# jkflying/opencalibration

Measured on AMD Instinct MI355X. Metric: images/sec end-to-end (extract+match+relax) on synthetic aerial grid; LM iters/sec, higher is better.
Workload: dtype f32 (extract) + fp4 0/1 bits, f32 accumulate, exact (match) + f64 (RANSAC, relax)

## Files before the change

opencalibration_amd/capi.py:

```python
import ctypes as C
import os

import numpy as np

_HERE = os.path.dirname(os.path.abspath(__file__))
LIB_PATH = os.path.join(_HERE, "libochip.so")

K_MATCH, K_RANSAC, K_RELAX_EVAL, K_RELAX_SOLVE, K_AKAZE = 0, 1, 2, 3, 4
NO_SECOND = 0xFFFF

PAIR_DTYPE = np.dtype([("image_1", np.uint32), ("image_2", np.uint32)])
MATCH_DTYPE = np.dtype([("best_k", np.uint32), ("best_count", np.uint16), ("second_count", np.uint16)])
RANSAC_JOB_DTYPE = np.dtype([("image_1", np.uint32), ("image_2", np.uint32), ("n", np.uint32), ("rng_state", np.uint32),
                             ("match_offset", np.uint64), ("eval_offset", np.uint64)])
RANSAC_MATCH_DTYPE = np.dtype([("k1", np.uint32), ("k2", np.uint32), ("count", np.uint16), ("reserved", np.uint16)])
RANSAC_RESULT_DTYPE = np.dtype([("H", np.float64, (9,)), ("score", np.float64), ("iterations", np.uint32), ("n_inliers", np.uint32),
                                ("improvements", np.uint32), ("reserved", np.uint32)])

EXPORTS = [
    "ochip_ctx_create", "ochip_ctx_destroy", "ochip_ctx_sibling", "ochip_ctx_attachment", "ochip_akaze_progress", "ochip_ctx_set_priority", "ochip_last_error", "ochip_device_info", "ochip_synchronize",
    "ochip_descriptors_reserve", "ochip_upload_descriptors", "ochip_descriptor_count",
    "ochip_match_batch", "ochip_match_launch", "ochip_match_fetch",
    "ochip_upload_keypoints", "ochip_ransac_homography_batch", "ochip_refit_homography_batch", "ochip_ransac_epipolar_batch",
    "ochip_upload_batch", "ochip_host_alloc", "ochip_host_free", "ochip_akaze_batch", "ochip_akaze_batch_dev", "ochip_akaze_features", "ochip_akaze_features_dev", "ochip_feature_lists_from_keypoints",
# ... 285 lines not shown

    def std_sort(self, keys, payload, offsets):
        keys = np.ascontiguousarray(keys, np.uint32)
        payload = np.ascontiguousarray(payload, np.uint32)
        offsets = np.ascontiguousarray(offsets, np.uint32)
        n_segs = len(offsets) - 1
        ko, po = np.zeros(max(len(keys), 1), np.uint32), np.zeros(max(len(keys), 1), np.uint32)
        fb = np.zeros(max(n_segs, 1), np.uint8)
        kin = keys if len(keys) else np.zeros(1, np.uint32)
        pin = payload if len(keys) else np.zeros(1, np.uint32)
        self._check(self.L.ochip_debug_std_sort(self.h, kin.ctypes.data, pin.ctypes.data, offsets.ctypes.data, n_segs, ko.ctypes.data,
                                                po.ctypes.data, fb.ctypes.data), "ochip_debug_std_sort")
        return ko[:len(keys)], po[:len(keys)], fb[:n_segs].astype(bool)

    def feature_lists(self, kp6, desc, work_wh, scale, nms_radius=8.0, subset_spacing=0.0):
        kp6 = np.ascontiguousarray(kp6, np.float32).reshape(-1, 6)
        desc = np.ascontiguousarray(desc, np.uint64).reshape(-1, 8)
        n = len(kp6)
        m = max(n, 1)
        rec, resp = np.zeros((m + 1, 88), np.uint8), np.zeros(m, np.float32)
        slot, ns, conflict = np.zeros(m, np.uint32), np.zeros(4, np.uint32), np.zeros(16, np.uint8)
        subset, nsub, sconf = np.zeros(16384, np.uint32), np.zeros(4, np.uint32), np.zeros(16, np.uint8)
        counts = np.array([n], np.uint32)

        class Lists(C.Structure):
            _fields_ = [("records", C.c_void_p), ("response", C.c_void_p), ("slot", C.c_void_p), ("num_sparse", C.c_void_p),
                        ("conflict", C.c_void_p), ("subset", C.c_void_p), ("num_subset", C.c_void_p), ("subset_conflict", C.c_void_p),
                        ("subset_spacing", C.c_double)]

        lists = Lists(rec.ctypes.data, resp.ctypes.data, slot.ctypes.data, ns.ctypes.data, conflict.ctypes.data, subset.ctypes.data,
                      nsub.ctypes.data, sconf.ctypes.data, float(subset_spacing))
        kin = kp6 if n else np.zeros((1, 6), np.float32)
        din = desc if n else np.zeros((1, 8), np.uint64)
        self._check(self.L.ochip_feature_lists_from_keypoints(self.h, kin.ctypes.data, din.ctypes.data, counts.ctypes.data, 1, m,
                                                              int(work_wh[0]), int(work_wh[1]), float(scale), float(nms_radius),
                                                              C.byref(lists)), "ochip_feature_lists_from_keypoints")
        out = dict(records=rec[:n + 1 if n else 0], response=resp[:n], slot=slot[:n], num_sparse=int(ns[0]), conflict=bool(conflict[0]))
        if subset_spacing > 0:
            out.update(subset=subset[:int(nsub[0])].copy(), subset_conflict=bool(sconf[0]))
        return out

    def synth_views(self, position, orientation, width, height, f, pp, plane, spacing, origin, seed=7, chunk=64):
        n = len(position)
        ptr = C.c_void_p()
        self._check(self.L.ochip_synth_views_alloc(self.h, n, width, height, C.byref(ptr)), "ochip_synth_views_alloc")
        cams = np.ascontiguousarray(np.concatenate([position, orientation], axis=1), np.float64)
        model3 = np.array([f, pp[0], pp[1]], np.float64)
        plane2 = np.array(plane, np.float64)
        lat3 = np.array([origin[0], origin[1], spacing], np.float64)
        for i in range(0, n, chunk):
            m = min(chunk, n - i)
            c = np.ascontiguousarray(cams[i:i + m])
            self._check(self.L.ochip_synth_render_views(self.h, ptr, i, m, width, height, c.ctypes.data, model3.ctypes.data,
                                                        plane2.ctypes.data, lat3.ctypes.data, seed), "ochip_synth_render_views")
        return ptr.value
# ... 195 lines not shown
```

opencalibration_amd/csrc/akaze.hip:

```cpp
#include "ctx.hpp"

#include <algorithm>
#include <cmath>
#include <limits>
#include <cstring>
#include <type_traits>
#include <vector>

namespace
{

struct level_info
{
    int octave, w, h, sigma_size;
    float esigma;
    size_t off;
    int tile_off, tiles_x;
    int mask_off;
    int sup_off, sup_tx;
};

__device__ __forceinline__ int clampi(int v, int lo, int hi)
{
    return v < lo ? lo : (v > hi ? hi : v);
}
__device__ __forceinline__ int reflect101_once(int v, int n)
{
    v = v < 0 ? -v : v;
    return v >= n ? 2 * (n - 1) - v : v;
}
__device__ __forceinline__ int reflect101(int v, int n)
// ... 740 lines not shown
__global__ void copy_plane_kernel(const float *__restrict__ in, size_t in_stride, float *__restrict__ out,
                                  size_t out_stride, size_t n)
{
    const size_t i = (size_t)blockIdx.x * blockDim.x + threadIdx.x;
    if (i < n)
        out[(size_t)blockIdx.z * out_stride + i] = in[(size_t)blockIdx.z * in_stride + i];
}

struct cand_t
{
    int level, x, y;
    float response;
    float dx, dy;
};

template <int S>
__global__ __launch_bounds__(256) void det_maxima_kernel(const float2 *__restrict__ Lxy, size_t stride,
                                                         float2 *__restrict__ Fit, float *__restrict__ Rmax, int w, int h,
                                                         float thr, unsigned int *__restrict__ tile_counts, int tile_off,
                                                         int n_tiles, float margin, unsigned long long *__restrict__ mask,
                                                         size_t mask_stride)
{
    constexpr int HW = S + 1, RW = BT_X + 2 * HW, RH = DT_Y + 2 * HW, DW = BT_X + 2, DH = DT_Y + 2;
    __shared__ float tx[RW * RH], ty[RW * RH];
    static_assert(DW * DH <= RW * RH, "the determinant tile reuses the Lx tile's storage");
    float *td = tx;
    const int tiles_x = (w + BT_X - 1) / BT_X, tiles_y = (h + DT_Y - 1) / DT_Y;
    int tile_x, tile_y;
    if (!xcd_tile(tiles_x, tiles_y, &tile_x, &tile_y))
        return;
    const int x0 = tile_x * BT_X, y0 = tile_y * DT_Y;
    const int rx0 = x0 - HW, ry0 = y0 - HW;
    const float2 *XY = Lxy + (size_t)blockIdx.z * stride;
// ... 154 lines not shown
                            mx = false;
                if (mx)
                {
                    out = v;
                    const float vxp = td[ci + 1], vxm = td[ci - 1], vyp = td[ci + DW], vym = td[ci - DW];
                    const float Dx = 0.5f * (vxp - vxm), Dy = 0.5f * (vyp - vym);
                    const float Dxx = (vxp + vxm) - 2.0f * v, Dyy = (vyp + vym) - 2.0f * v;
                    const float Dxy = 0.25f * ((td[ci + DW + 1] + td[ci - DW - 1]) - (td[ci + DW - 1] + td[ci - DW + 1]));
                    fit = subpixel_solve(Dxx, Dxy, Dyy, Dx, Dy);
                }
            }
        }
        const unsigned long long m = __ballot(out != 0.0f);
        if (out != 0.0f)
        {
            Rmax[(size_t)blockIdx.z * stride + (size_t)y * w + x] = out;
            Fit[(size_t)blockIdx.z * stride + (size_t)y * w + x] = fit;
        }
        if (lx == 0 && y < h)
        {
            mask[(size_t)blockIdx.z * mask_stride + (size_t)y * tiles_x + tile_x] = m;
            found += (unsigned int)__popcll(m);
        }
    }
    __shared__ unsigned int wsum[4];
    for (int off = 32; off >= 1; off >>= 1)
        found += (unsigned int)__shfl_xor((int)found, off);
    if ((threadIdx.x & 63) == 0)
        wsum[threadIdx.x >> 6] = found;
    __syncthreads();
    if (threadIdx.x == 0)
        tile_counts[(size_t)blockIdx.z * n_tiles + tile_off + tile_y * tiles_x + tile_x] =
// ... 21 lines not shown
__device__ __forceinline__ float max2f(float a, float b)
{
    float r;
    asm("v_max_f32 %0, %1, %2" : "=v"(r) : "v"(a), "v"(b));
    return r;
}
__device__ __forceinline__ float2 subpixel_fit(float v, float vxm, float vxp, float vym, float vyp, float vmm, float vpm, float vmp, float vpp)
{
    const float Dx = 0.5f * (vxp - vxm), Dy = 0.5f * (vyp - vym);
    const float Dxx = (vxp + vxm) - 2.0f * v, Dyy = (vyp + vym) - 2.0f * v;
    const float Dxy = 0.25f * ((vpp + vmm) - (vmp + vpm));
    return subpixel_solve(Dxx, Dxy, Dyy, Dx, Dy);
}

template <int S>
__global__ __launch_bounds__(256) void det_strip_kernel(const float2 *__restrict__ Lxy, size_t stride, float2 *__restrict__ Fit,
                                                        float *__restrict__ Rmax, int w, int h, float thr,
                                                        unsigned int *__restrict__ tile_counts, int tile_off, int n_tiles,
                                                        int4 win ,
                                                        unsigned long long *__restrict__ mask, size_t mask_stride)
{
    typedef float pk2 __attribute__((ext_vector_type(2)));
    typedef det_strip_geom<S> G;
    constexpr int HALO = G::HALO, OW = G::OW, U = G::U, RB = G::RB, NB = G::NB, SH = G::H;
    constexpr int LROW = 128 + 2 * DS_PAD;
    __shared__ __attribute__((aligned(16))) float ex[4][3][LROW];
    const int lane = threadIdx.x & 63, wv = __builtin_amdgcn_readfirstlane(threadIdx.x >> 6);
    const int strips_x = (w + OW - 1) / OW, strips_y = (h + SH - 1) / SH;
    const int groups = (strips_x * strips_y + 3) / 4, chunk = (groups + 7) / 8;
    const int g = (int)(blockIdx.x & 7) * chunk + (int)(blockIdx.x >> 3);
    if ((int)(blockIdx.x >> 3) >= chunk || g >= groups)
        return;
// ... 32 lines not shown
    float DL[U], DR[U];
#pragma unroll
    for (int j = 0; j < U; j++)
    {
        X[j] = Y[j] = pa_hd[j] = pb_hd[j] = D[j] = T[j] = Sd[j] = pk2{0.0f, 0.0f};
        DL[j] = DR[j] = 0.0f;
    }
    __shared__ float4 notes[4][DS_NOTES][3];
    unsigned int n_noted = 0;
    auto flush_notes = [&](unsigned int n) {
        wave_sync();
        if ((unsigned int)lane < n)
        {
            const float4 r0 = notes[wv][lane][0], r1 = notes[wv][lane][1], r2 = notes[wv][lane][2];
            const int x = __float_as_int(r0.x), y = __float_as_int(r0.y);
            const size_t at = (size_t)blockIdx.z * stride + (size_t)y * w + x;
            Rmax[at] = r0.z;
            Fit[at] = subpixel_fit(r0.z, r0.w, r1.x, r1.y, r1.z, r1.w, r2.x, r2.y, r2.z);
            atomicOr(&mask[(size_t)blockIdx.z * mask_stride + (size_t)y * tiles_x + (x >> 6)], 1ull << (x & 63));
            atomicAdd(&tile_counts[(size_t)blockIdx.z * n_tiles + tile_off + (y / DT_Y) * tiles_x + (x >> 6)], 1u);
        }
        wave_sync();
    };
    for (int k = 0; k < NB; k++)
    {
#pragma unroll
        for (int jj = 0; jj < RB; jj++)
        {
            const int r = k * RB + jj;
            constexpr int UU = U;
            const int j = jj % UU;
            const int s_top = (j + 1) % UU, s_c = (j + S + 1) % UU, s_m = (j + S) % UU, s_mm = (j + S - 1) % UU;
            request(r + PF, (jj + PF) % RB);
// ... 398 lines not shown
        unsigned int base = carry;
        for (int j = 0; j < wv; j++)
            base += wsum[j];
        if (i < n_tiles)
            tile_base[(size_t)b * n_tiles + tile] = base + incl - v;
        __syncthreads();
        if (threadIdx.x == 0)
            carry += wsum[0] + wsum[1] + wsum[2] + wsum[3];
        __syncthreads();
    }
    if (threadIdx.x == 0)
        n_cands[b] = carry;
}

constexpr int COLLECT_TPW = 4;
__global__ __launch_bounds__(256) void collect_tiles_kernel(const float *__restrict__ Rmax, const float2 *__restrict__ Fit,
                                                            size_t img_stride,
                                                            const unsigned long long *__restrict__ mask, size_t mask_stride,
                                                            levels_dev L, const unsigned int *__restrict__ tile_base, int n_tiles,
                                                            cand_t *__restrict__ cands, unsigned int max_cands,
                                                            const unsigned int *__restrict__ tile_counts)
{
    static_assert(2 * DT_Y <= 64, "two tiles' rows per wavefront");
    const unsigned int b = blockIdx.z;
    const int lane = threadIdx.x & 63, half = lane >= DT_Y ? 1 : 0, row = lane - half * DT_Y;
    const int first = (blockIdx.x * 4 + (int)(threadIdx.x >> 6)) * COLLECT_TPW;
    for (int pair = 0; pair < COLLECT_TPW; pair += 2)
    {
        if (first + pair >= n_tiles)
            break;
        const int tile = first + pair + half;
        bool live = lane < 2 * DT_Y && tile < n_tiles;
        live = live && tile_counts[(size_t)b * n_tiles + tile] != 0;
        if (__ballot(live) == 0)
            continue;
        int level = 0;
        while (level + 1 < L.n && tile >= L.l[level + 1].tile_off)
            level++;
        const level_info l = L.l[level];
        const int t = tile - l.tile_off;
        const int ty = t / l.tiles_x, tx = t - ty * l.tiles_x;
        const float *R = Rmax + (size_t)b * img_stride + l.off;
        const float2 *F = Fit + (size_t)b * img_stride + l.off;
        const int y = ty * DT_Y + row;
        unsigned long long m = 0;
        if (live && y < l.h)
            m = mask[(size_t)b * mask_stride + (size_t)l.mask_off + (size_t)y * l.tiles_x + tx];
        const unsigned int cnt = (unsigned int)__popcll(m);
        unsigned int incl = cnt;
        for (int off = 1; off < 64; off <<= 1)
        {
            const unsigned int v = (unsigned int)__shfl_up((int)incl, off);
            if (lane >= off)
                incl += v;
        }
        const unsigned int first_total = (unsigned int)__builtin_amdgcn_readlane((int)incl, DT_Y - 1);
        unsigned int slot = (live ? tile_base[(size_t)b * n_tiles + tile] : 0u) + incl - cnt - (half ? first_total : 0u);
        while (m)
        {
            const int bit = __ffsll((long long)m) - 1;
            m &= m - 1;
            const int x = tx * BT_X + bit;
            if (slot < max_cands)
            {
                const float2 f = F[(size_t)y * l.w + x];
                cands[(size_t)b * max_cands + slot] = cand_t{level, x, y, R[(size_t)y * l.w + x], f.x, f.y};
            }
            slot++;
        }
    }
}

__device__ __forceinline__ bool xcd_contiguous(unsigned int block, unsigned int n_items, unsigned int *item, int mode)
{
    if (mode == 0)
    {
        *item = block;
        return block < n_items;
    }
    const unsigned int x = block & 7, j = block >> 3;
    if (mode == 1)
// ... 187 lines not shown
            const int r = PASS == 2 ? l.sigma_size * diff : lo.sigma_size;
            const int px = PASS == 2 ? c.x * diff : c.x >> shift, py = PASS == 2 ? c.y * diff : c.y >> shift;
            int fx = 0, fy = 0;
            if (sup_first_set(own + (size_t)b * mask_stride + lo.sup_off, lo, px, py, r, &fx, &fy, (hooks & 1) != 0))
            {
                f = (unsigned int)fx | ((unsigned int)fy << 16) | SUP_FOUND;
                atomicOr(&has[word], bit);
            }
        }
    }
    found[(size_t)b * max_cands + k] = f;
}

template <int PASS>
__global__ __launch_bounds__(256) void suppress_round0_kernel(const cand_t *__restrict__ cands, const unsigned int *__restrict__ n_cands,
                                                              unsigned int max_cands, const float *__restrict__ Rmax, size_t img_stride,
                                                              const unsigned long long *__restrict__ own, unsigned long long *pend,
                                                              unsigned long long *kmask, size_t mask_stride, levels_dev L,
                                                              const unsigned int *__restrict__ level_first,
                                                              unsigned int *__restrict__ turns, unsigned int *__restrict__ waiting,
                                                              const unsigned int *__restrict__ found, int hooks)
{
    const unsigned int b = blockIdx.z, k = blockIdx.x * 256 + threadIdx.x, n = min(n_cands[b], max_cands);
    cand_t c = cand_t{0, 0, 0, 0.f, 0.f, 0.f};
    bool has_turn = k < n;
    unsigned int f = 0;
    if (has_turn)
    {
        if (PASS != 1)
        {
            f = found[(size_t)b * max_cands + k];
// ... 10 lines not shown
        const level_info l = one_level ? L.l[lv0] : L.l[c.level];
        const size_t word = (size_t)b * mask_stride + (size_t)l.sup_off + sup_word(l, c.x, c.y);
        const unsigned long long bit = sup_bit(c.x, c.y);
        const int other = PASS == 1 ? 0 : (PASS == 2 ? -1 : 1);
        const level_info lo = one_level ? L.l[lv0 + other] : L.l[c.level + other];
        const int shift = PASS == 3 ? lo.octave - l.octave : 0;
        const int box = PASS == 3 ? 2 * lo.sigma_size * (1 << shift) - 1 : 2 * l.sigma_size - 1;
        waits = sup_pending(own + (size_t)b * mask_stride + l.sup_off, l, c.x, c.y, box, (hooks & 1) != 0);
        if (waits)
            atomicOr(&pend[word], bit);
        else if (PASS == 1)
            atomicOr(&kmask[word], bit);
        else
        {
            const int fx = (int)(f & 0xffffu), fy = (int)((f & ~SUP_FOUND) >> 16);
            if (c.response > Rmax[(size_t)b * img_stride + lo.off + (size_t)fy * lo.w + fx])
                atomicAnd(&kmask[(size_t)b * mask_stride + lo.sup_off + sup_word(lo, fx, fy)], ~sup_bit(fx, fy));
        }
    }
    const int lane = threadIdx.x & 63;
    unsigned long long todo = __ballot(waits);
    while (todo)
    {
        const int leader = __ffsll((long long)todo) - 1;
        const int lv = __builtin_amdgcn_readlane(c.level, leader);
        const unsigned long long same = __ballot(waits && c.level == lv);
        unsigned int base = 0;
        if (lane == leader)
            base = atomicAdd(&waiting[(size_t)b * L.n + lv], (unsigned int)__popcll(same));
        base = (unsigned int)__builtin_amdgcn_readlane((int)base, leader);
        if (waits && c.level == lv)
            turns[(size_t)b * 2 * max_cands + level_first[(size_t)b * (L.n + 1) + lv] + base +
                  (unsigned int)__popcll(same & ((1ull << lane) - 1ull))] = (unsigned int)c.x | ((unsigned int)c.y << 16);
        todo &= ~same;
    }
}

template <int PASS>
__global__ __launch_bounds__(SUP_THREADS) void suppress_rounds_kernel(const unsigned int *__restrict__ n_cands, unsigned int max_cands,
                                                                      const float *__restrict__ Rmax, size_t img_stride,
                                                                      unsigned long long *pend, unsigned long long *kmask, size_t mask_stride,
                                                                      levels_dev L, const unsigned int *__restrict__ level_first,
                                                                      unsigned int *turns, unsigned int *waiting, unsigned int *__restrict__ stats,
                                                                      int hooks)
{
    const unsigned int b = blockIdx.x, tid = threadIdx.x;
    const int level = (int)blockIdx.y + (PASS == 2 ? 1 : 0);
    const unsigned int m0 = waiting[(size_t)b * L.n + level];
    if (m0 == 0)
        return;
    const long long t_begin = stats ? (long long)wall_clock64() : 0;
    const unsigned int first = level_first[(size_t)b * (L.n + 1) + level];
    const level_info l = L.l[level], lo = L.l[PASS == 1 ? level : (PASS == 2 ? level - 1 : level + 1)];
    unsigned long long *Pm = pend + (size_t)b * mask_stride + l.sup_off, *W = kmask + (size_t)b * mask_stride + l.sup_off,
                       *Wo = kmask + (size_t)b * mask_stride + lo.sup_off;
    const float *R = Rmax + (size_t)b * img_stride + l.off, *Ro = Rmax + (size_t)b * img_stride + lo.off;
    const int diff = PASS == 2 ? 1 << (l.octave - lo.octave) : 1, shift = PASS == 3 ? lo.octave - l.octave : 0;
    const int box = PASS == 3 ? 2 * lo.sigma_size * (1 << shift) - 1 : 2 * l.sigma_size - 1;
    const int r = PASS == 1 ? l.sigma_size : (PASS == 2 ? l.sigma_size * diff : lo.sigma_size);
    __shared__ unsigned int s_list[2][SUP_LDS];
    __shared__ unsigned int s_n[2];
    unsigned int *spill0 = turns + (size_t)b * 2 * max_cands + first, *spill1 = spill0 + max_cands;
    const unsigned int in_lds = (hooks & 2) ? 64u : (unsigned int)SUP_LDS;
    auto get = [&](int which, unsigned int idx) { return idx < in_lds ? s_list[which][idx] : (which ? spill1 : spill0)[idx]; };
    auto put = [&](int which, unsigned int idx, unsigned int v) {
        if (idx < in_lds)
            s_list[which][idx] = v;
        else
            (which ? spill1 : spill0)[idx] = v;
    };
    for (unsigned int idx = tid; idx < min(m0, in_lds); idx += SUP_THREADS)
// ... 16 lines not shown
            if (!sup_pending(Pm, l, (int)(e & 0xffffu), (int)(e >> 16), box, (hooks & 1) != 0))
                put(cur, idx, e | SUP_READY);
        }
        __syncthreads();
        for (unsigned int idx = tid; idx < m; idx += SUP_THREADS)
        {
            const unsigned int e = get(cur, idx);
            if (!(e & SUP_READY))
            {
                put(cur ^ 1, atomicAdd(&s_n[cur ^ 1], 1u), e);
                continue;
            }
            const int x = (int)(e & 0xffffu), y = (int)((e & ~SUP_READY) >> 16);
            const size_t word = sup_word(l, x, y);
            const unsigned long long bit = sup_bit(x, y);
            const float response = R[(size_t)y * l.w + x];
            int fx = 0, fy = 0;
            if (PASS == 1)
            {
                bool keep = true;
                if (sup_first_set(W, l, x, y, r, &fx, &fy, (hooks & 1) != 0))
                {
                    if (response > R[(size_t)fy * l.w + fx])
                        atomicAnd(&W[sup_word(l, fx, fy)], ~sup_bit(fx, fy));
                    else
                        keep = false;
                }
                if (keep)
                    atomicOr(&W[word], bit);
            }
            else
            {
                const int px = PASS == 2 ? x * diff : x >> shift, py = PASS == 2 ? y * diff : y >> shift;
                if (sup_first_set(Wo, lo, px, py, r, &fx, &fy, (hooks & 1) != 0) && response > Ro[(size_t)fy * lo.w + fx])
                    atomicAnd(&Wo[sup_word(lo, fx, fy)], ~sup_bit(fx, fy));
            }
            atomicAnd(&Pm[word], ~bit);
        }
        __syncthreads();
        cur ^= 1;
    }
    if (tid == 0)
    {
        waiting[(size_t)b * L.n + level] = 0;
        if (stats)
        {
            unsigned int *o = stats + (((size_t)(PASS - 1) * gridDim.x + b) * L.n + level) * 3;
            o[0] = rounds, o[1] = (unsigned int)((long long)wall_clock64() - t_begin), o[2] = m0;
        }
// ... 932 lines not shown
    if (work_wh)
    {
        work_wh[0] = W;
        work_wh[1] = H;
    }
    for (uint32_t i = 0; i < n_images; i++)
        counts[i] = 0;
    if (n_images == 0)
        return OCHIP_OK;

    const int omax = 4, nsub = 4;
    const float soffset = 1.6f, dfactor = 1.5f, dthreshold = 0.00005f;
    levels_dev LV{};
    std::vector<std::vector<float>> tsteps;
    size_t img_stride = 0;
    int n_tiles = 0;
    size_t mask_stride = 0;
    size_t sup_stride = 0;
    {
        std::vector<float> etime;
        for (int i = 0; i < omax; i++)
        {
            const float rfactor = 1.0f / (float)(1 << i);
            const int lw = (int)(W * rfactor), lh = (int)(H * rfactor);
            if ((lw < 80 || lh < 40) && i != 0)
                break;
            for (int j = 0; j < nsub; j++)
            {
                level_info &l = LV.l[LV.n++];
                l.octave = i;
                l.w = lw;
                l.h = lh;
                l.esigma = soffset * std::pow(2.0f, (float)j / (float)nsub + (float)i);
                l.sigma_size = (int)std::lrintf(l.esigma * dfactor / (float)(1 << i));
                l.off = img_stride;
                img_stride += (size_t)lw * lh;
                l.tiles_x = (lw + BT_X - 1) / BT_X;
                l.tile_off = n_tiles;
                n_tiles += l.tiles_x * ((lh + DT_Y - 1) / DT_Y);
                l.mask_off = (int)mask_stride;
                mask_stride += (size_t)l.tiles_x * lh;
                l.sup_off = (int)sup_stride;
                l.sup_tx = (lw + 7) / 8;
                sup_stride += (size_t)l.sup_tx * ((lh + 7) / 8);
                etime.push_back(0.5f * (l.esigma * l.esigma));
            }
        }
        tsteps.resize(LV.n);
        for (int i = 1; i < LV.n; i++)
            tsteps[i] = fed_taus(etime[i] - etime[i - 1], 0.25f);
    }
// ... 5 lines not shown
    auto cleanup = [&]() {
        (void)ochip_stream_wait(ctx, st);
        for (auto &a : allocs)
            ochip_pool_put(ctx, a.first, a.second);
    };
    int rc = OCHIP_OK;
#define AK(call)                                                                                                       \
    do                                                                                                                 \
    {                                                                                                                  \
        if (rc == OCHIP_OK)                                                                                            \
            rc = (call);                                                                                               \
    } while (0)
    uint8_t *d_bgr = nullptr, *d_gray = nullptr;
    float *d_img = nullptr, *d_flow = nullptr, *d_ping = nullptr;
    float2 *d_Lxy = nullptr;
    float2 *d_Fit = nullptr;
    float *d_Lt = nullptr, *d_Rmax = nullptr, *d_kc = nullptr,
          *d_kp = nullptr;
    unsigned int *d_hmax = nullptr, *d_hist = nullptr, *d_ncand = nullptr, *d_pmax = nullptr;
    cand_t *d_cands = nullptr;
    unsigned char *d_dead = nullptr, *d_valid = nullptr;
    unsigned long long *d_desc = nullptr, *d_descc = nullptr;
    float *d_kpc = nullptr;
    unsigned int *d_counts = nullptr, *d_tile_counts = nullptr, *d_tile_base = nullptr, *d_tile_seq = nullptr;
    unsigned long long *d_mask = nullptr, *d_vmask = nullptr, *d_kmask = nullptr, *d_pmask = nullptr, *d_rmask = nullptr;
    unsigned int *d_found = nullptr;
    unsigned int *d_level_first = nullptr;
    unsigned int *d_turns = nullptr, *d_waiting = nullptr;
    unsigned int *d_wbase = nullptr, *d_live = nullptr, *d_nlive = nullptr;
    gather_tab *d_gtab = nullptr;
    const size_t src_px = (size_t)width * height;
    auto tiles = [&](int w, int h) { return dim3(8 * ((((w + BT_X - 1) / BT_X) * ((h + BT_Y - 1) / BT_Y) + 7) / 8), 1, B); };
    auto det_tiles = [&](int w, int h) { return dim3(8 * ((((w + BT_X - 1) / BT_X) * ((h + DT_Y - 1) / DT_Y) + 7) / 8), 1, B); };
    const dim3 tiles0 = tiles(W, H);
    const int n_tiles0 = ((W + BT_X - 1) / BT_X) * ((H + BT_Y - 1) / BT_Y);
    if (on_device)
        d_bgr = const_cast<uint8_t *>(images_bgr);
    else
        AK(up(ctx, allocs, &d_bgr, images_bgr, (size_t)B * src_px * 3));
    AK(up<uint8_t>(ctx, allocs, &d_gray, nullptr, (size_t)B * src_px + 4));
    AK(up<float>(ctx, allocs, &d_img, nullptr, (size_t)B * plane0));
    AK(up<float>(ctx, allocs, &d_flow, nullptr, (size_t)B * plane0));
    AK(up<float>(ctx, allocs, &d_ping, nullptr, (size_t)B * plane0));
    AK(up<unsigned int>(ctx, allocs, &d_pmax, nullptr, (size_t)B * n_tiles0));
    AK(up<float>(ctx, allocs, &d_Lt, nullptr, (size_t)B * img_stride));
    AK(up<float2>(ctx, allocs, &d_Lxy, nullptr, (size_t)B * img_stride));
    AK(up<float2>(ctx, allocs, &d_Fit, nullptr, (size_t)B * img_stride));
    AK(up<float>(ctx, allocs, &d_Rmax, nullptr, (size_t)B * img_stride));
    AK(up<float>(ctx, allocs, &d_kc, nullptr, B));
    AK(up<unsigned int>(ctx, allocs, &d_hmax, nullptr, B));
    AK(up<unsigned int>(ctx, allocs, &d_hist, nullptr, (size_t)B * 301));
    AK(up<unsigned int>(ctx, allocs, &d_ncand, nullptr, B));
    AK(up<cand_t>(ctx, allocs, &d_cands, nullptr, (size_t)B * max_cands));
    AK(up<unsigned char>(ctx, allocs, &d_dead, nullptr, (size_t)B * max_cands));
    AK(up<unsigned char>(ctx, allocs, &d_valid, nullptr, (size_t)B * max_cands));
    AK(up<float>(ctx, allocs, &d_kp, nullptr, (size_t)B * max_cands * 6));
    AK(up<unsigned long long>(ctx, allocs, &d_desc, nullptr, (size_t)B * max_cands * 8));
    AK(up<float>(ctx, allocs, &d_kpc, nullptr, (size_t)B * max_kp * 6));
    AK(up<unsigned long long>(ctx, allocs, &d_descc, nullptr, (size_t)B * max_kp * 8));
    AK(up<unsigned int>(ctx, allocs, &d_counts, nullptr, B));
    AK(up<unsigned int>(ctx, allocs, &d_tile_counts, nullptr, (size_t)B * n_tiles));
    AK(up<unsigned int>(ctx, allocs, &d_tile_base, nullptr, (size_t)B * n_tiles));
    AK(up<unsigned long long>(ctx, allocs, &d_mask, nullptr, (size_t)B * mask_stride));
// ... 386 lines not shown
            blur_args a{d_Lt + l.off, img_stride, (float *)(d_Lxy + l.off), nullptr, img_stride, l.w, l.h, nullptr, 0, nullptr, nullptr, 0};
            if (l.sigma_size == 2)
                hipLaunchKernelGGL((blur_fused_kernel<BLUR_DERIV, 2, 0>), tiles(l.w, l.h), dim3(256), 0, st, a, one);
            else if (l.sigma_size == 3)
                hipLaunchKernelGGL((blur_fused_kernel<BLUR_DERIV, 3, 0>), tiles(l.w, l.h), dim3(256), 0, st, a, one);
            else if (l.sigma_size == 4)
                hipLaunchKernelGGL((blur_fused_kernel<BLUR_DERIV, 4, 0>), tiles(l.w, l.h), dim3(256), 0, st, a, one);
            else
            {
                cleanup();
                return ochip_fail(ctx, OCHIP_EINVAL, "akaze: derivative scale %d outside 2..4", l.sigma_size);
            }
        }
        {
            const float2 *lxy = d_Lxy + l.off;
            float2 *ld = d_Fit + l.off;
            float *rm = d_Rmax + l.off;
            const float margin = (10.0f * std::sqrt(2.0f)) * (float)l.sigma_size;
            const int4 win = det_window(l);
            auto strip_grid = [&](int ow, int sh) {
                const int strips = ((l.w + ow - 1) / ow) * ((l.h + sh - 1) / sh);
                return dim3(8 * (((strips + 3) / 4 + 7) / 8), 1, B);
            };
            const bool det_strip = det_strips && strips_pay(l, force_det_strips);
            if (det_strip && l.sigma_size == 2)
                hipLaunchKernelGGL((det_strip_kernel<2>), strip_grid(det_strip_geom<2>::OW, det_strip_geom<2>::H), dim3(256), 0, st, lxy, img_stride, ld, rm, l.w,
                                   l.h, dthreshold, d_tile_counts, l.tile_off, n_tiles, win, d_mask + l.mask_off, mask_stride);
            else if (det_strip && l.sigma_size == 3)
                hipLaunchKernelGGL((det_strip_kernel<3>), strip_grid(det_strip_geom<3>::OW, det_strip_geom<3>::H), dim3(256), 0, st, lxy, img_stride, ld, rm, l.w,
                                   l.h, dthreshold, d_tile_counts, l.tile_off, n_tiles, win, d_mask + l.mask_off, mask_stride);
            else if (det_strip)
                hipLaunchKernelGGL((det_strip_kernel<4>), strip_grid(det_strip_geom<4>::OW, det_strip_geom<4>::H), dim3(256), 0, st, lxy, img_stride, ld, rm, l.w,
                                   l.h, dthreshold, d_tile_counts, l.tile_off, n_tiles, win, d_mask + l.mask_off, mask_stride);
            else if (l.sigma_size == 2)
                hipLaunchKernelGGL((det_maxima_kernel<2>), det_tiles(l.w, l.h), dim3(256), 0, st, lxy, img_stride, ld, rm, l.w,
                                   l.h, dthreshold, d_tile_counts, l.tile_off, n_tiles, margin, d_mask + l.mask_off, mask_stride);
            else if (l.sigma_size == 3)
                hipLaunchKernelGGL((det_maxima_kernel<3>), det_tiles(l.w, l.h), dim3(256), 0, st, lxy, img_stride, ld, rm, l.w,
                                   l.h, dthreshold, d_tile_counts, l.tile_off, n_tiles, margin, d_mask + l.mask_off, mask_stride);
            else
                hipLaunchKernelGGL((det_maxima_kernel<4>), det_tiles(l.w, l.h), dim3(256), 0, st, lxy, img_stride, ld, rm, l.w,
                                   l.h, dthreshold, d_tile_counts, l.tile_off, n_tiles, margin, d_mask + l.mask_off, mask_stride);
        }
    }
    if (const char *dump = std::getenv("OCHIP_DUMP_PLANES"))
    {
        std::vector<float> hl(img_stride), hx(2 * img_stride);
        OCHIP_HIP(ctx, ochip_stream_wait(ctx, st));
        OCHIP_HIP(ctx, hipMemcpy(hl.data(), d_Lt, img_stride * 4, hipMemcpyDeviceToHost));
        OCHIP_HIP(ctx, hipMemcpy(hx.data(), d_Lxy, img_stride * 8, hipMemcpyDeviceToHost));
        for (int which = 0; which < 2; which++)
            if (FILE *f = std::fopen((std::string(dump) + (which ? "_lxy.f32" : "_lt.f32")).c_str(), "wb"))
            {
                std::fwrite(which ? hx.data() : hl.data(), 4, which ? hx.size() : hl.size(), f);
                std::fclose(f);
            }
    }
    hipLaunchKernelGGL(scan_tiles_kernel, dim3(B), dim3(256), 0, st, (const unsigned int *)d_tile_counts,
                       (const unsigned int *)d_tile_seq, n_tiles, d_tile_base, d_ncand);
    hipLaunchKernelGGL(collect_tiles_kernel, dim3((n_tiles + 4 * COLLECT_TPW - 1) / (4 * COLLECT_TPW), 1, B), dim3(256), 0, st, (const float *)d_Rmax,
                       (const float2 *)d_Fit, img_stride,
                       (const unsigned long long *)d_mask, mask_stride, LV, (const unsigned int *)d_tile_base, n_tiles, d_cands,
                       max_cands, (const unsigned int *)d_tile_counts);
    std::vector<unsigned int> ncand(B);
    OCHIP_HIP(ctx, hipMemcpyAsync(ncand.data(), d_ncand, B * 4, hipMemcpyDeviceToHost, st));
    OCHIP_HIP(ctx, ochip_stream_wait(ctx, st));
    ctx->akaze_readbacks.fetch_add(1, std::memory_order_release);
    unsigned int max_n = 0;
    for (uint32_t b = 0; b < B; b++)
    {
        if (ncand[b] > max_cands)
        {
            cleanup();
            return ochip_fail(ctx, OCHIP_ENOMEM, "image %u has %u extrema candidates; raise max_kp (candidate capacity %u)", b,
                              ncand[b], max_cands);
        }
// ... 8 lines not shown
        unsigned int *d_sup_stats = nullptr;
        if (ochip_verbose("extract"))
        {
            AK(up<unsigned int>(ctx, allocs, &d_sup_stats, nullptr, (size_t)3 * B * LV.n * 3));
            OCHIP_HIP(ctx, hipMemsetAsync(d_sup_stats, 0, (size_t)3 * B * LV.n * 3 * 4, st));
        }
        OCHIP_HIP(ctx, hipMemsetAsync(d_kmask, 0, (size_t)B * sup_stride * 8, st));
        OCHIP_HIP(ctx, hipMemsetAsync(d_pmask, 0, (size_t)B * sup_stride * 8, st));
        OCHIP_HIP(ctx, hipMemsetAsync(d_waiting, 0, (size_t)B * LV.n * 4, st));
        hipLaunchKernelGGL(suppress_level_first_kernel, dim3(B), dim3(64), 0, st, (const unsigned int *)d_ncand, max_cands, LV,
                           (const unsigned int *)d_tile_base, (const unsigned int *)d_tile_seq, n_tiles, d_level_first);
        hipLaunchKernelGGL(suppress_tiles_kernel, dim3((unsigned int)((LV.l[0].tiles_x * ((LV.l[0].h + 7) / 8) + 255) / 256), LV.n, B),
                           dim3(256), 0, st, (const unsigned long long *)d_mask, mask_stride, d_rmask, sup_stride, LV);
#define SUP_PASS(PASS, LEVELS)                                                                                                                 \
    hipLaunchKernelGGL(suppress_round0_kernel<PASS>, per_cand, dim3(256), 0, st, (const cand_t *)d_cands, (const unsigned int *)d_ncand,       \
                       max_cands, (const float *)d_Rmax, img_stride, (const unsigned long long *)d_rmask, d_pmask, d_kmask, sup_stride, LV,    \
                       (const unsigned int *)d_level_first, d_turns, d_waiting, (const unsigned int *)d_found, sup_hooks);                     \
    hipLaunchKernelGGL(suppress_rounds_kernel<PASS>, dim3(B, (LEVELS)), dim3(SUP_THREADS), 0, st, (const unsigned int *)d_ncand, max_cands,    \
                       (const float *)d_Rmax, img_stride, d_pmask, d_kmask, sup_stride, LV, (const unsigned int *)d_level_first, d_turns,      \
                       d_waiting, d_sup_stats, sup_hooks)
#define SUP_WINDOWS(PASS)                                                                                                                      \
    OCHIP_HIP(ctx, hipMemsetAsync(d_rmask, 0, (size_t)B * sup_stride * 8, st));                                                                \
    hipLaunchKernelGGL(suppress_window_kernel<PASS>, per_cand, dim3(256), 0, st, (const cand_t *)d_cands, (const unsigned int *)d_ncand,       \
                       max_cands, (const unsigned long long *)d_kmask, d_rmask, sup_stride, LV, d_found, sup_hooks)
        SUP_PASS(1, LV.n);
        if (LV.n > 1)
        {
            SUP_WINDOWS(2);
            SUP_PASS(2, LV.n - 1);
            SUP_WINDOWS(3);
            SUP_PASS(3, LV.n - 1);
        }
#undef SUP_WINDOWS
        hipLaunchKernelGGL(suppress_dead_kernel, per_cand, dim3(256), 0, st, (const cand_t *)d_cands, (const unsigned int *)d_ncand,
// ... 84 lines not shown
```

opencalibration_amd/csrc/features.hip:

```cpp
#include "ctx.hpp"

#include <algorithm>
#include <cstdlib>
#include <cstring>
#include <vector>

using namespace ochip;

namespace
{

enum : unsigned char
{
    UNDECIDED = 0,
    SPARSE = 1,
    DENSE = 2
};

struct nms_dev
{
    unsigned int B, S;
    const unsigned int *n;
    const double2 *loc;
    double cell, scale2, radius2;
// ... 116 lines not shown
__global__ void nms_fill_kernel(nms_dev N)
{
    const unsigned int b = blockIdx.z, r = blockIdx.x * blockDim.x + threadIdx.x;
    if (r >= N.n[b])
        return;
    const size_t o = (size_t)b * N.S + r;
    const int n_cells = N.gw * N.gh;
    const unsigned int c = N.cell_id[o];
    const unsigned int at = N.cell_start[(size_t)b * (n_cells + 1) + c] + atomicAdd(&N.cell_fill[(size_t)b * n_cells + c], 1u);
    N.items[(size_t)b * N.S + at] = r;
    N.item_loc[(size_t)b * N.S + at] = N.loc[o];
    N.state[o] = UNDECIDED;
}

template <typename StateOf>
__device__ __forceinline__ unsigned char nms_decide(const nms_dev &N, unsigned int b, unsigned int r, StateOf state_of)
{
    const size_t base = (size_t)b * N.S;
    const int n_cells = N.gw * N.gh;
    const unsigned int *start = N.cell_start + (size_t)b * (n_cells + 1);
    const unsigned int *items = N.items + base;
    const double2 *item_loc = N.item_loc + base;
    const double2 me = N.loc[base + r];
    const int c = (int)N.cell_id[base + r], cx = c % N.gw, cy = c / N.gw;
    bool open_near = false;
    for (int yy = max(cy - 1, 0); yy <= min(cy + 1, N.gh - 1); yy++)
    {
        const unsigned int i0 = start[yy * N.gw + max(cx - 1, 0)], i1 = start[yy * N.gw + min(cx + 1, N.gw - 1) + 1];
        for (unsigned int i = i0; i < i1; i++)
        {
            const unsigned int q = items[i];
            if (q >= r)
                continue;
            if (!nms_within(N, me, item_loc[i]))
                continue;
            const unsigned char sq = state_of(q);
            if (sq == SPARSE)
                return DENSE;
            if (sq == UNDECIDED)
                open_near = true;
        }
    }
    return open_near ? UNDECIDED : SPARSE;
}

__global__ void nms_round_kernel(nms_dev N)
{
    const unsigned int b = blockIdx.z, r = blockIdx.x * blockDim.x + threadIdx.x;
    if (r >= N.n[b])
        return;
    unsigned char *st = N.state + (size_t)b * N.S;
    if (st[r] != UNDECIDED)
        return;
    const unsigned char s = nms_decide(N, b, r, [&](unsigned int q) { return st[q]; });
    if (s != UNDECIDED)
        st[r] = s;
}

constexpr int FIN_THREADS = 256;
template <bool SUBSET> __global__ __launch_bounds__(FIN_THREADS) void nms_finish_kernel(nms_dev N, feat_dev F)
{
    extern __shared__ unsigned char state[];
    __shared__ unsigned int s_scan[FIN_THREADS];
    __shared__ int s_again;
    const unsigned int b = blockIdx.x, t = threadIdx.x;
    const unsigned int n = N.n[b];
    const size_t base = (size_t)b * N.S;
    if (t == 0)
        s_again = 0;
    for (unsigned int r = t; r < n; r += FIN_THREADS)
        state[r] = N.state[base + r];
    __syncthreads();
    for (;;)
    {
        bool any_left = false;
        for (unsigned int r = t; r < n; r += FIN_THREADS)
        {
            if (state[r] != UNDECIDED)
                continue;
            const unsigned char s = nms_decide(N, b, r, [&](unsigned int q) { return state[q]; });
            if (s != UNDECIDED)
                state[r] = s;
            else
                any_left = true;
        }
        if (any_left)
            s_again = 1;
        __syncthreads();
        const int again = s_again;
        __syncthreads();
        if (t == 0)
            s_again = 0;
        if (!again)
            break;
        __syncthreads();
// ... 300 lines not shown
```

Measured before the change: 3912.

## Pack detector maxima into half-resolution float4 records and iterate NMS in cell order

Replaces the full-resolution Rmax and Fit planes with one packed float4 record per 2x2 pixel block, written by the detector kernels and read by collect and suppression. This cuts the memory footprint and the strided scattered reads, on the assumption that at most one maximum falls in each 2x2 block. NMS threads now walk candidates in cell-sorted order and recompute the cell from the location, which improves locality. The Python wrapper gains a batched feature_lists path that handles several images in one call.

```diff
diff --git a/opencalibration_amd/capi.py b/opencalibration_amd/capi.py
--- a/opencalibration_amd/capi.py
+++ b/opencalibration_amd/capi.py
@@ -323,14 +323,20 @@
         return ko[:len(keys)], po[:len(keys)], fb[:n_segs].astype(bool)
 
     def feature_lists(self, kp6, desc, work_wh, scale, nms_radius=8.0, subset_spacing=0.0):
-        kp6 = np.ascontiguousarray(kp6, np.float32).reshape(-1, 6)
-        desc = np.ascontiguousarray(desc, np.uint64).reshape(-1, 8)
-        n = len(kp6)
-        m = max(n, 1)
-        rec, resp = np.zeros((m + 1, 88), np.uint8), np.zeros(m, np.float32)
-        slot, ns, conflict = np.zeros(m, np.uint32), np.zeros(4, np.uint32), np.zeros(16, np.uint8)
-        subset, nsub, sconf = np.zeros(16384, np.uint32), np.zeros(4, np.uint32), np.zeros(16, np.uint8)
-        counts = np.array([n], np.uint32)
+        return self.feature_lists_batch([(kp6, desc)], work_wh, scale, nms_radius, subset_spacing)[0]
+
+    def feature_lists_batch(self, images, work_wh, scale, nms_radius=8.0, subset_spacing=0.0):
+        images = [(np.ascontiguousarray(k, np.float32).reshape(-1, 6), np.ascontiguousarray(d, np.uint64).reshape(-1, 8))
+                  for k, d in images]
+        B = len(images)
+        m = max([len(k) for k, _ in images] + [1])
+        kin, din = np.zeros((B, m, 6), np.float32), np.zeros((B, m, 8), np.uint64)
+        for i, (k, d) in enumerate(images):
+            kin[i, :len(k)], din[i, :len(k)] = k, d
+        counts = np.array([len(k) for k, _ in images], np.uint32)
+        rec, resp = np.zeros((B, m + 1, 88), np.uint8), np.zeros((B, m), np.float32)
+        slot, ns, conflict = np.zeros((B, m), np.uint32), np.zeros(B + 4, np.uint32), np.zeros(B + 16, np.uint8)
+        subset, nsub, sconf = np.zeros((B, 16384), np.uint32), np.zeros(B + 4, np.uint32), np.zeros(B + 16, np.uint8)
 
         class Lists(C.Structure):
             _fields_ = [("records", C.c_void_p), ("response", C.c_void_p), ("slot", C.c_void_p), ("num_sparse", C.c_void_p),
@@ -339,15 +345,18 @@
 
         lists = Lists(rec.ctypes.data, resp.ctypes.data, slot.ctypes.data, ns.ctypes.data, conflict.ctypes.data, subset.ctypes.data,
                       nsub.ctypes.data, sconf.ctypes.data, float(subset_spacing))
-        kin = kp6 if n else np.zeros((1, 6), np.float32)
-        din = desc if n else np.zeros((1, 8), np.uint64)
-        self._check(self.L.ochip_feature_lists_from_keypoints(self.h, kin.ctypes.data, din.ctypes.data, counts.ctypes.data, 1, m,
+        self._check(self.L.ochip_feature_lists_from_keypoints(self.h, kin.ctypes.data, din.ctypes.data, counts.ctypes.data, B, m,
                                                               int(work_wh[0]), int(work_wh[1]), float(scale), float(nms_radius),
                                                               C.byref(lists)), "ochip_feature_lists_from_keypoints")
-        out = dict(records=rec[:n + 1 if n else 0], response=resp[:n], slot=slot[:n], num_sparse=int(ns[0]), conflict=bool(conflict[0]))
-        if subset_spacing > 0:
-            out.update(subset=subset[:int(nsub[0])].copy(), subset_conflict=bool(sconf[0]))
-        return out
+        outs = []
+        for i, (k, _) in enumerate(images):
+            n = len(k)
+            out = dict(records=rec[i, :n + 1 if n else 0].copy(), response=resp[i, :n].copy(), slot=slot[i, :n].copy(),
+                       num_sparse=int(ns[i]), conflict=bool(conflict[i]))
+            if subset_spacing > 0:
+                out.update(subset=subset[i, :int(nsub[i])].copy(), subset_conflict=bool(sconf[i]))
+            outs.append(out)
+        return outs
 
     def synth_views(self, position, orientation, width, height, f, pp, plane, spacing, origin, seed=7, chunk=64):
         n = len(position)
diff --git a/opencalibration_amd/csrc/akaze.hip b/opencalibration_amd/csrc/akaze.hip
--- a/opencalibration_amd/csrc/akaze.hip
+++ b/opencalibration_amd/csrc/akaze.hip
@@ -15,6 +15,8 @@
     int octave, w, h, sigma_size;
     float esigma;
     size_t off;
+    size_t rec_off;
+    int rec_w;
     int tile_off, tiles_x;
     int mask_off;
     int sup_off, sup_tx;
@@ -785,9 +787,14 @@
     float dx, dy;
 };
 
+__device__ __forceinline__ size_t max_rec_at(int rec_w, int x, int y)
+{
+    return (size_t)(y >> 1) * rec_w + (x >> 1);
+}
+
 template <int S>
 __global__ __launch_bounds__(256) void det_maxima_kernel(const float2 *__restrict__ Lxy, size_t stride,
-                                                         float2 *__restrict__ Fit, float *__restrict__ Rmax, int w, int h,
+                                                         float4 *__restrict__ Rec, size_t rec_stride, int rec_w, int w, int h,
                                                          float thr, unsigned int *__restrict__ tile_counts, int tile_off,
                                                          int n_tiles, float margin, unsigned long long *__restrict__ mask,
                                                          size_t mask_stride)
@@ -972,8 +979,7 @@
         const unsigned long long m = __ballot(out != 0.0f);
         if (out != 0.0f)
         {
-            Rmax[(size_t)blockIdx.z * stride + (size_t)y * w + x] = out;
-            Fit[(size_t)blockIdx.z * stride + (size_t)y * w + x] = fit;
+            Rec[(size_t)blockIdx.z * rec_stride + max_rec_at(rec_w, x, y)] = make_float4(out, fit.x, fit.y, 0.0f);
         }
         if (lx == 0 && y < h)
         {
@@ -1025,8 +1031,8 @@
 }
 
 template <int S>
-__global__ __launch_bounds__(256) void det_strip_kernel(const float2 *__restrict__ Lxy, size_t stride, float2 *__restrict__ Fit,
-                                                        float *__restrict__ Rmax, int w, int h, float thr,
+__global__ __launch_bounds__(256) void det_strip_kernel(const float2 *__restrict__ Lxy, size_t stride, float4 *__restrict__ Rec,
+                                                        size_t rec_stride, int rec_w, int w, int h, float thr,
                                                         unsigned int *__restrict__ tile_counts, int tile_off, int n_tiles,
                                                         int4 win ,
                                                         unsigned long long *__restrict__ mask, size_t mask_stride)
@@ -1089,9 +1095,8 @@
         {
             const float4 r0 = notes[wv][lane][0], r1 = notes[wv][lane][1], r2 = notes[wv][lane][2];
             const int x = __float_as_int(r0.x), y = __float_as_int(r0.y);
-            const size_t at = (size_t)blockIdx.z * stride + (size_t)y * w + x;
-            Rmax[at] = r0.z;
-            Fit[at] = subpixel_fit(r0.z, r0.w, r1.x, r1.y, r1.z, r1.w, r2.x, r2.y, r2.z);
+            const float2 fit = subpixel_fit(r0.z, r0.w, r1.x, r1.y, r1.z, r1.w, r2.x, r2.y, r2.z);
+            Rec[(size_t)blockIdx.z * rec_stride + max_rec_at(rec_w, x, y)] = make_float4(r0.z, fit.x, fit.y, 0.0f);
             atomicOr(&mask[(size_t)blockIdx.z * mask_stride + (size_t)y * tiles_x + (x >> 6)], 1ull << (x & 63));
             atomicAdd(&tile_counts[(size_t)blockIdx.z * n_tiles + tile_off + (y / DT_Y) * tiles_x + (x >> 6)], 1u);
         }
@@ -1520,8 +1525,7 @@
 }
 
 constexpr int COLLECT_TPW = 4;
-__global__ __launch_bounds__(256) void collect_tiles_kernel(const float *__restrict__ Rmax, const float2 *__restrict__ Fit,
-                                                            size_t img_stride,
+__global__ __launch_bounds__(256) void collect_tiles_kernel(const float4 *__restrict__ Rec, size_t rec_stride,
                                                             const unsigned long long *__restrict__ mask, size_t mask_stride,
                                                             levels_dev L, const unsigned int *__restrict__ tile_base, int n_tiles,
                                                             cand_t *__restrict__ cands, unsigned int max_cands,
@@ -1546,8 +1550,7 @@
         const level_info l = L.l[level];
         const int t = tile - l.tile_off;
         const int ty = t / l.tiles_x, tx = t - ty * l.tiles_x;
-        const float *R = Rmax + (size_t)b * img_stride + l.off;
-        const float2 *F = Fit + (size_t)b * img_stride + l.off;
+        const float4 *M = Rec + (size_t)b * rec_stride + l.rec_off;
         const int y = ty * DT_Y + row;
         unsigned long long m = 0;
         if (live && y < l.h)
@@ -1569,8 +1572,8 @@
             const int x = tx * BT_X + bit;
             if (slot < max_cands)
             {
-                const float2 f = F[(size_t)y * l.w + x];
-                cands[(size_t)b * max_cands + slot] = cand_t{level, x, y, R[(size_t)y * l.w + x], f.x, f.y};
+                const float4 r = M[max_rec_at(l.rec_w, x, y)];
+                cands[(size_t)b * max_cands + slot] = cand_t{level, x, y, r.x, r.y, r.z};
             }
             slot++;
         }
@@ -1788,7 +1791,7 @@
 
 template <int PASS>
 __global__ __launch_bounds__(256) void suppress_round0_kernel(const cand_t *__restrict__ cands, const unsigned int *__restrict__ n_cands,
-                                                              unsigned int max_cands, const float *__restrict__ Rmax, size_t img_stride,
+                                                              unsigned int max_cands, const float4 *__restrict__ Rec, size_t rec_stride,
                                                               const unsigned long long *__restrict__ own, unsigned long long *pend,
                                                               unsigned long long *kmask, size_t mask_stride, levels_dev L,
                                                               const unsigned int *__restrict__ level_first,
@@ -1829,7 +1832,7 @@
         else
         {
             const int fx = (int)(f & 0xffffu), fy = (int)((f & ~SUP_FOUND) >> 16);
-            if (c.response > Rmax[(size_t)b * img_stride + lo.off + (size_t)fy * lo.w + fx])
+            if (c.response > Rec[(size_t)b * rec_stride + lo.rec_off + max_rec_at(lo.rec_w, fx, fy)].x)
                 atomicAnd(&kmask[(size_t)b * mask_stride + lo.sup_off + sup_word(lo, fx, fy)], ~sup_bit(fx, fy));
         }
     }
@@ -1853,7 +1856,7 @@
 
 template <int PASS>
 __global__ __launch_bounds__(SUP_THREADS) void suppress_rounds_kernel(const unsigned int *__restrict__ n_cands, unsigned int max_cands,
-                                                                      const float *__restrict__ Rmax, size_t img_stride,
+                                                                      const float4 *__restrict__ Rec, size_t rec_stride,
                                                                       unsigned long long *pend, unsigned long long *kmask, size_t mask_stride,
                                                                       levels_dev L, const unsigned int *__restrict__ level_first,
                                                                       unsigned int *turns, unsigned int *waiting, unsigned int *__restrict__ stats,
@@ -1869,7 +1872,7 @@
     const level_info l = L.l[level], lo = L.l[PASS == 1 ? level : (PASS == 2 ? level - 1 : level + 1)];
     unsigned long long *Pm = pend + (size_t)b * mask_stride + l.sup_off, *W = kmask + (size_t)b * mask_stride + l.sup_off,
                        *Wo = kmask + (size_t)b * mask_stride + lo.sup_off;
-    const float *R = Rmax + (size_t)b * img_stride + l.off, *Ro = Rmax + (size_t)b * img_stride + lo.off;
+    const float4 *R = Rec + (size_t)b * rec_stride + l.rec_off, *Ro = Rec + (size_t)b * rec_stride + lo.rec_off;
     const int diff = PASS == 2 ? 1 << (l.octave - lo.octave) : 1, shift = PASS == 3 ? lo.octave - l.octave : 0;
     const int box = PASS == 3 ? 2 * lo.sigma_size * (1 << shift) - 1 : 2 * l.sigma_size - 1;
     const int r = PASS == 1 ? l.sigma_size : (PASS == 2 ? l.sigma_size * diff : lo.sigma_size);
@@ -1916,14 +1919,14 @@
             const int x = (int)(e & 0xffffu), y = (int)((e & ~SUP_READY) >> 16);
             const size_t word = sup_word(l, x, y);
             const unsigned long long bit = sup_bit(x, y);
-            const float response = R[(size_t)y * l.w + x];
+            const float response = R[max_rec_at(l.rec_w, x, y)].x;
             int fx = 0, fy = 0;
             if (PASS == 1)
             {
                 bool keep = true;
                 if (sup_first_set(W, l, x, y, r, &fx, &fy, (hooks & 1) != 0))
                 {
-                    if (response > R[(size_t)fy * l.w + fx])
+                    if (response > R[max_rec_at(l.rec_w, fx, fy)].x)
                         atomicAnd(&W[sup_word(l, fx, fy)], ~sup_bit(fx, fy));
                     else
                         keep = false;
@@ -1934,7 +1937,7 @@
             else
             {
                 const int px = PASS == 2 ? x * diff : x >> shift, py = PASS == 2 ? y * diff : y >> shift;
-                if (sup_first_set(Wo, lo, px, py, r, &fx, &fy, (hooks & 1) != 0) && response > Ro[(size_t)fy * lo.w + fx])
+                if (sup_first_set(Wo, lo, px, py, r, &fx, &fy, (hooks & 1) != 0) && response > Ro[max_rec_at(lo.rec_w, fx, fy)].x)
                     atomicAnd(&Wo[sup_word(lo, fx, fy)], ~sup_bit(fx, fy));
             }
             atomicAnd(&Pm[word], ~bit);
@@ -2897,6 +2900,7 @@
     levels_dev LV{};
     std::vector<std::vector<float>> tsteps;
     size_t img_stride = 0;
+    size_t rec_stride = 0;
     int n_tiles = 0;
     size_t mask_stride = 0;
     size_t sup_stride = 0;
@@ -2918,6 +2922,9 @@
                 l.sigma_size = (int)std::lrintf(l.esigma * dfactor / (float)(1 << i));
                 l.off = img_stride;
                 img_stride += (size_t)lw * lh;
+                l.rec_off = rec_stride;
+                l.rec_w = (lw + 1) / 2;
+                rec_stride += (size_t)l.rec_w * ((lh + 1) / 2);
                 l.tiles_x = (lw + BT_X - 1) / BT_X;
                 l.tile_off = n_tiles;
                 n_tiles += l.tiles_x * ((lh + DT_Y - 1) / DT_Y);
@@ -2953,8 +2960,8 @@
     uint8_t *d_bgr = nullptr, *d_gray = nullptr;
     float *d_img = nullptr, *d_flow = nullptr, *d_ping = nullptr;
     float2 *d_Lxy = nullptr;
-    float2 *d_Fit = nullptr;
-    float *d_Lt = nullptr, *d_Rmax = nullptr, *d_kc = nullptr,
+    float4 *d_Rec = nullptr;
+    float *d_Lt = nullptr, *d_kc = nullptr,
           *d_kp = nullptr;
     unsigned int *d_hmax = nullptr, *d_hist = nullptr, *d_ncand = nullptr, *d_pmax = nullptr;
     cand_t *d_cands = nullptr;
@@ -2984,8 +2991,7 @@
     AK(up<unsigned int>(ctx, allocs, &d_pmax, nullptr, (size_t)B * n_tiles0));
     AK(up<float>(ctx, allocs, &d_Lt, nullptr, (size_t)B * img_stride));
     AK(up<float2>(ctx, allocs, &d_Lxy, nullptr, (size_t)B * img_stride));
-    AK(up<float2>(ctx, allocs, &d_Fit, nullptr, (size_t)B * img_stride));
-    AK(up<float>(ctx, allocs, &d_Rmax, nullptr, (size_t)B * img_stride));
+    AK(up<float4>(ctx, allocs, &d_Rec, nullptr, (size_t)B * rec_stride));
     AK(up<float>(ctx, allocs, &d_kc, nullptr, B));
     AK(up<unsigned int>(ctx, allocs, &d_hmax, nullptr, B));
     AK(up<unsigned int>(ctx, allocs, &d_hist, nullptr, (size_t)B * 301));
@@ -3402,8 +3408,7 @@
         }
         {
             const float2 *lxy = d_Lxy + l.off;
-            float2 *ld = d_Fit + l.off;
-            float *rm = d_Rmax + l.off;
+            float4 *rec = d_Rec + l.rec_off;
             const float margin = (10.0f * std::sqrt(2.0f)) * (float)l.sigma_size;
             const int4 win = det_window(l);
             auto strip_grid = [&](int ow, int sh) {
@@ -3412,22 +3417,22 @@
             };
             const bool det_strip = det_strips && strips_pay(l, force_det_strips);
             if (det_strip && l.sigma_size == 2)
-                hipLaunchKernelGGL((det_strip_kernel<2>), strip_grid(det_strip_geom<2>::OW, det_strip_geom<2>::H), dim3(256), 0, st, lxy, img_stride, ld, rm, l.w,
+                hipLaunchKernelGGL((det_strip_kernel<2>), strip_grid(det_strip_geom<2>::OW, det_strip_geom<2>::H), dim3(256), 0, st, lxy, img_stride, rec, rec_stride, l.rec_w, l.w,
                                    l.h, dthreshold, d_tile_counts, l.tile_off, n_tiles, win, d_mask + l.mask_off, mask_stride);
             else if (det_strip && l.sigma_size == 3)
-                hipLaunchKernelGGL((det_strip_kernel<3>), strip_grid(det_strip_geom<3>::OW, det_strip_geom<3>::H), dim3(256), 0, st, lxy, img_stride, ld, rm, l.w,
+                hipLaunchKernelGGL((det_strip_kernel<3>), strip_grid(det_strip_geom<3>::OW, det_strip_geom<3>::H), dim3(256), 0, st, lxy, img_stride, rec, rec_stride, l.rec_w, l.w,
                                    l.h, dthreshold, d_tile_counts, l.tile_off, n_tiles, win, d_mask + l.mask_off, mask_stride);
             else if (det_strip)
-                hipLaunchKernelGGL((det_strip_kernel<4>), strip_grid(det_strip_geom<4>::OW, det_strip_geom<4>::H), dim3(256), 0, st, lxy, img_stride, ld, rm, l.w,
+                hipLaunchKernelGGL((det_strip_kernel<4>), strip_grid(det_strip_geom<4>::OW, det_strip_geom<4>::H), dim3(256), 0, st, lxy, img_stride, rec, rec_stride, l.rec_w, l.w,
                                    l.h, dthreshold, d_tile_counts, l.tile_off, n_tiles, win, d_mask + l.mask_off, mask_stride);
             else if (l.sigma_size == 2)
-                hipLaunchKernelGGL((det_maxima_kernel<2>), det_tiles(l.w, l.h), dim3(256), 0, st, lxy, img_stride, ld, rm, l.w,
+                hipLaunchKernelGGL((det_maxima_kernel<2>), det_tiles(l.w, l.h), dim3(256), 0, st, lxy, img_stride, rec, rec_stride, l.rec_w, l.w,
                                    l.h, dthreshold, d_tile_counts, l.tile_off, n_tiles, margin, d_mask + l.mask_off, mask_stride);
             else if (l.sigma_size == 3)
-                hipLaunchKernelGGL((det_maxima_kernel<3>), det_tiles(l.w, l.h), dim3(256), 0, st, lxy, img_stride, ld, rm, l.w,
+                hipLaunchKernelGGL((det_maxima_kernel<3>), det_tiles(l.w, l.h), dim3(256), 0, st, lxy, img_stride, rec, rec_stride, l.rec_w, l.w,
                                    l.h, dthreshold, d_tile_counts, l.tile_off, n_tiles, margin, d_mask + l.mask_off, mask_stride);
             else
-                hipLaunchKernelGGL((det_maxima_kernel<4>), det_tiles(l.w, l.h), dim3(256), 0, st, lxy, img_stride, ld, rm, l.w,
+                hipLaunchKernelGGL((det_maxima_kernel<4>), det_tiles(l.w, l.h), dim3(256), 0, st, lxy, img_stride, rec, rec_stride, l.rec_w, l.w,
                                    l.h, dthreshold, d_tile_counts, l.tile_off, n_tiles, margin, d_mask + l.mask_off, mask_stride);
         }
     }
@@ -3446,8 +3451,8 @@
     }
     hipLaunchKernelGGL(scan_tiles_kernel, dim3(B), dim3(256), 0, st, (const unsigned int *)d_tile_counts,
                        (const unsigned int *)d_tile_seq, n_tiles, d_tile_base, d_ncand);
-    hipLaunchKernelGGL(collect_tiles_kernel, dim3((n_tiles + 4 * COLLECT_TPW - 1) / (4 * COLLECT_TPW), 1, B), dim3(256), 0, st, (const float *)d_Rmax,
-                       (const float2 *)d_Fit, img_stride,
+    hipLaunchKernelGGL(collect_tiles_kernel, dim3((n_tiles + 4 * COLLECT_TPW - 1) / (4 * COLLECT_TPW), 1, B), dim3(256), 0, st, (const float4 *)d_Rec,
+                       rec_stride,
                        (const unsigned long long *)d_mask, mask_stride, LV, (const unsigned int *)d_tile_base, n_tiles, d_cands,
                        max_cands, (const unsigned int *)d_tile_counts);
     std::vector<unsigned int> ncand(B);
@@ -3486,10 +3491,10 @@
                            dim3(256), 0, st, (const unsigned long long *)d_mask, mask_stride, d_rmask, sup_stride, LV);
 #define SUP_PASS(PASS, LEVELS)                                                                                                                 \
     hipLaunchKernelGGL(suppress_round0_kernel<PASS>, per_cand, dim3(256), 0, st, (const cand_t *)d_cands, (const unsigned int *)d_ncand,       \
-                       max_cands, (const float *)d_Rmax, img_stride, (const unsigned long long *)d_rmask, d_pmask, d_kmask, sup_stride, LV,    \
+                       max_cands, (const float4 *)d_Rec, rec_stride, (const unsigned long long *)d_rmask, d_pmask, d_kmask, sup_stride, LV,    \
                        (const unsigned int *)d_level_first, d_turns, d_waiting, (const unsigned int *)d_found, sup_hooks);                     \
     hipLaunchKernelGGL(suppress_rounds_kernel<PASS>, dim3(B, (LEVELS)), dim3(SUP_THREADS), 0, st, (const unsigned int *)d_ncand, max_cands,    \
-                       (const float *)d_Rmax, img_stride, d_pmask, d_kmask, sup_stride, LV, (const unsigned int *)d_level_first, d_turns,      \
+                       (const float4 *)d_Rec, rec_stride, d_pmask, d_kmask, sup_stride, LV, (const unsigned int *)d_level_first, d_turns,      \
                        d_waiting, d_sup_stats, sup_hooks)
 #define SUP_WINDOWS(PASS)                                                                                                                      \
     OCHIP_HIP(ctx, hipMemsetAsync(d_rmask, 0, (size_t)B * sup_stride * 8, st));                                                                \
diff --git a/opencalibration_amd/csrc/features.hip b/opencalibration_amd/csrc/features.hip
--- a/opencalibration_amd/csrc/features.hip
+++ b/opencalibration_amd/csrc/features.hip
@@ -154,15 +154,15 @@
 }
 
 template <typename StateOf>
-__device__ __forceinline__ unsigned char nms_decide(const nms_dev &N, unsigned int b, unsigned int r, StateOf state_of)
+__device__ __forceinline__ unsigned char nms_decide(const nms_dev &N, unsigned int b, unsigned int at, unsigned int r, StateOf state_of)
 {
     const size_t base = (size_t)b * N.S;
     const int n_cells = N.gw * N.gh;
     const unsigned int *start = N.cell_start + (size_t)b * (n_cells + 1);
     const unsigned int *items = N.items + base;
     const double2 *item_loc = N.item_loc + base;
-    const double2 me = N.loc[base + r];
-    const int c = (int)N.cell_id[base + r], cx = c % N.gw, cy = c / N.gw;
+    const double2 me = item_loc[at];
+    const int cx = min(max((int)(me.x / N.cell), 0), N.gw - 1), cy = min(max((int)(me.y / N.cell), 0), N.gh - 1);
     bool open_near = false;
     for (int yy = max(cy - 1, 0); yy <= min(cy + 1, N.gh - 1); yy++)
     {
@@ -186,13 +186,14 @@
 
 __global__ void nms_round_kernel(nms_dev N)
 {
-    const unsigned int b = blockIdx.z, r = blockIdx.x * blockDim.x + threadIdx.x;
-    if (r >= N.n[b])
+    const unsigned int b = blockIdx.z, i = blockIdx.x * blockDim.x + threadIdx.x;
+    if (i >= N.n[b])
         return;
     unsigned char *st = N.state + (size_t)b * N.S;
+    const unsigned int r = N.items[(size_t)b * N.S + i];
     if (st[r] != UNDECIDED)
         return;
-    const unsigned char s = nms_decide(N, b, r, [&](unsigned int q) { return st[q]; });
+    const unsigned char s = nms_decide(N, b, i, r, [&](unsigned int q) { return st[q]; });
     if (s != UNDECIDED)
         st[r] = s;
 }
@@ -214,11 +215,12 @@
     for (;;)
     {
         bool any_left = false;
-        for (unsigned int r = t; r < n; r += FIN_THREADS)
+        for (unsigned int i = t; i < n; i += FIN_THREADS)
         {
+            const unsigned int r = N.items[base + i];
             if (state[r] != UNDECIDED)
                 continue;
-            const unsigned char s = nms_decide(N, b, r, [&](unsigned int q) { return state[q]; });
+            const unsigned char s = nms_decide(N, b, i, r, [&](unsigned int q) { return state[q]; });
             if (s != UNDECIDED)
                 state[r] = s;
             else
```

Measured after the change: 3906. About the same (-0.2%).
